# kernel-matrix-benchmarks/kernel-matrix-benchmarks

Measured on AMD Instinct MI355X. Metric: point-pair interactions/s (N*M/s) + max |err| vs scipy, D=3 Gaussian, higher is better.
Workload: dtype f32

## Files before the change

kernel_matrix_benchmarks_amd/csrc/kmvp_api.hip:

```cpp
#include "kmvp_ctx.hpp"

namespace kmvp {

Rccl g_rccl;

namespace {
thread_local std::string g_create_error;
}

int fail(kmvp_ctx* c, int code, const std::string& msg) {
  if (c) c->err = msg;
  else g_create_error = msg;
  return code;
}
const char* create_error() { return g_create_error.c_str(); }

int ensure(kmvp_ctx* c, DevBuf& b, size_t bytes) {
  if (bytes <= b.cap && b.p) return KMVP_OK;
  if (b.p) {
    HIP_TRY(c, hipFree(b.p));
    b.p = nullptr;
    b.cap = 0;
  }
  if (bytes == 0) bytes = 16;
// ... 237 lines not shown
  ncclResult_t r = g_rccl.GetUniqueId(&id);
  if (r != ncclSuccess) return fail(nullptr, KMVP_E_COMM, std::string("ncclGetUniqueId: ") + g_rccl.GetErrorString(r));
  memcpy(id128, &id, sizeof(id));
  return KMVP_OK;
}

int kmvp_comm_init(kmvp_ctx* c, const void* id128, int rank, int world) {
  if (!c || !id128 || world < 1 || rank < 0 || rank >= world) return fail(c, KMVP_E_INVALID, "bad communicator arguments");
  if (!g_rccl.load()) return fail(c, KMVP_E_COMM, g_rccl.error);
  HIP_TRY(c, hipSetDevice(c->device));
  if (c->comm) {
    g_rccl.CommDestroy(c->comm);
    c->comm = nullptr;
  }
  c->host_xchg = nullptr;
  c->host_user = nullptr;
  ncclUniqueId id;
  memcpy(&id, id128, sizeof(id));
  ncclResult_t r = g_rccl.CommInitRank(&c->comm, world, id, rank);
  if (r != ncclSuccess) {
    c->comm = nullptr;
    return fail(c, KMVP_E_COMM, std::string("ncclCommInitRank: ") + g_rccl.GetErrorString(r));
  }
  int count = -1, user_rank = -1, dev = -1;
  ncclResult_t r1 = g_rccl.CommCount(c->comm, &count);
  ncclResult_t r2 = g_rccl.CommUserRank(c->comm, &user_rank);
  (void)g_rccl.CommCuDevice(c->comm, &dev);
  if (r1 != ncclSuccess || r2 != ncclSuccess || count != world || user_rank != rank) {
    g_rccl.CommDestroy(c->comm);
    c->comm = nullptr;
    c->comm_count = 1;
    c->rank = 0;
    c->world = 1;
    return fail(c, KMVP_E_COMM, "RCCL communicator mismatch: asked for rank " + std::to_string(rank) + " of " +
                                    std::to_string(world) + " on device " + std::to_string(c->device) + ", RCCL reports rank " +
                                    std::to_string(user_rank) + " of " + std::to_string(count) + " on device " +
                                    std::to_string(dev));
  }
  c->comm_count = count;
  c->rank = rank;
  c->world = world;
  return KMVP_OK;
}

int kmvp_comm_init_host(kmvp_ctx* c, kmvp_host_allreduce_fn fn, void* user, int rank, int world) {
  if (!c || !fn || world < 1 || rank < 0 || rank >= world) return fail(c, KMVP_E_INVALID, "bad communicator arguments");
  if (c->comm) {
    g_rccl.CommDestroy(c->comm);
    c->comm = nullptr;
  }
  c->host_xchg = fn;
  c->host_user = user;
  c->comm_count = world;
  c->rank = rank;
  c->world = world;
  return KMVP_OK;
}

int kmvp_comm_world(const kmvp_ctx* c) { return (c && c->exchanges()) ? c->comm_count : 1; }
int kmvp_comm_rank(const kmvp_ctx* c) { return (c && c->exchanges()) ? c->rank : 0; }

int kmvp_set_option(kmvp_ctx* c, const char* key, int64_t value) {
  if (!c || !key) return KMVP_E_INVALID;
  const std::string k(key);
  if (k == "feed") {
    if (value < -1 || value > 1) return fail(c, KMVP_E_INVALID, "feed must be -1 (auto), 0 or 1");
    c->opt_feed = (int)value;
  } else if (k == "targets_per_lane") {
    if (value != 0 && value != 1 && value != 2 && value != 4 && value != 8)
      return fail(c, KMVP_E_INVALID, "targets_per_lane must be 0 (auto), 1, 2, 4 or 8");
    c->opt_T = (int)value;
  } else if (k == "segments") {
    if (value < 0 || value > 65535) return fail(c, KMVP_E_INVALID, "segments out of range");
    c->opt_segments = (int)value;
  } else if (k == "fast_sqdists") {
    if (value < -1 || value > 4) return fail(c, KMVP_E_INVALID, "fast_sqdists must be -1 (auto), 0, 1, 2, 3 or 4");
    c->opt_fast = (int)value;
  } else if (k == "cellmm_shape") {
    if (value < -1 || value > 1) return fail(c, KMVP_E_INVALID, "cellmm_shape must be -1 (by size), 0 (32x32x16) or 1 (16x16x32)");
    c->opt_cellmm_shape = (int)value;
  } else if (k == "cell_fused") {
    if (value < -1 || value > 1) return fail(c, KMVP_E_INVALID, "cell_fused must be -1 (automatic), 0 (two launches) or 1 (one launch where it applies)");
    c->opt_cell_fused = (int)value;
  } else if (k == "mfma_variant") {
    if (value != -1 && value != 0 && value != 1 && value != 4 && value != 5)
      return fail(c, KMVP_E_INVALID, "mfma_variant must be -1 (by kernel), 0, 1, 4 or 5");
    c->opt_mfma_variant = (int)value;
  } else if (k == "same_points_global") {
    c->opt_same_global = value != 0;
  } else if (k == "partial_shard") {
    c->opt_partial = value != 0;
  } else if (k == "fast_tiles") {
    if (value != 0 && value != 1 && value != 2 && value != 4 && value != 8)
      return fail(c, KMVP_E_INVALID, "fast_tiles must be 0 (auto), 1, 2, 4 or 8");
    c->opt_fast_tiles = (int)value;
  } else if (k == "chunk") {
    if (value < 8 || value > (1 << 24)) return fail(c, KMVP_E_INVALID, "chunk out of range");
    c->opt_chunk = (int)value;
  } else {
    return fail(c, KMVP_E_INVALID, "unknown option " + k);
  }
  return KMVP_OK;
}

int64_t kmvp_device_bytes(const kmvp_ctx* c) {
  if (!c) return 0;
  size_t t = 0;
  for (const DevBuf* b : {&c->y_raw, &c->x_raw, &c->b_raw, &c->xs, &c->rec, &c->x_scaled,
                          &c->y_scaled, &c->part, &c->partd, &c->aux, &c->sortbuf, &c->perm, &c->sums, &c->out, &c->scratch, &c->sdiag, &c->xchg, &c->kexp, &c->kshift, &c->xchgk, &c->kflag,
                    &c->sk_xs_x, &c->sk_rec_y, &c->sk_xs_y, &c->sk_rec_x, &c->sk_state,
                          &c->cell_tperm, &c->cell_sperm, &c->cell_tgrp, &c->cell_sgrp, &c->cell_slot, &c->cell_tmeta, &c->cell_sums, &c->cell_skey, &c->cell_scentre, &c->cell_scale})
    t += b->cap;
  return (int64_t)t;
}
double kmvp_last_kernel_ms(const kmvp_ctx* c) { return c ? c->last_kernel_ms : 0.0; }
double kmvp_last_total_ms(const kmvp_ctx* c) { return c ? c->last_total_ms : 0.0; }
double kmvp_last_allreduce_ms(const kmvp_ctx* c) { return c ? c->last_allreduce_ms : 0.0; }
const char* kmvp_last_kernel_name(const kmvp_ctx* c) { return c ? c->last_kernel_name : ""; }
const char* kmvp_last_dispatch_note(const kmvp_ctx* c) { return c ? c->note.c_str() : ""; }

}
```

kernel_matrix_benchmarks_amd/csrc/kmvp_cellmm.hpp:

```cpp
#pragma once
#include <hip/hip_runtime.h>
#include <stdint.h>

#include "kmvp_cell.hpp"

namespace kmvp {

#ifndef CMM_BF16
#define CMM_BF16 0
#endif
#if CMM_BF16
typedef __bf16 cmm_half;
#else
typedef _Float16 cmm_half;
#endif
typedef cmm_half f16x8 __attribute__((ext_vector_type(8)));
typedef cmm_half f16x2 __attribute__((ext_vector_type(2)));

constexpr int CMM_STAGE_TILES = 12;
constexpr int CMM_STAGE_BYTES = 8192;
constexpr int CMM_E_OFF = 0;
constexpr int CMM_B_OFF = CMM_STAGE_TILES * CELL_TILE * 16;
constexpr int CMM_HDR_OFF = CMM_B_OFF + CMM_STAGE_TILES * CELL_TILE * 4;
static_assert(CMM_HDR_OFF + CMM_STAGE_TILES * 16 <= CMM_STAGE_BYTES, "stage image too small");
constexpr float CMM_TARGET_SCALE = 64.f;
constexpr int CMM_MAX_WLOG2 = 8;

struct CellmmArgs {
  const float* xd;
  const float* tmeta;
  const unsigned char* img;
  const float* scale;
  double* part;
  int64_t n_slots;
  int64_t tile_base;
  int64_t m_stages;
  int64_t seg_stages;
  int segments;
  int tile_blocks;
};

typedef int i32x4 __attribute__((ext_vector_type(4)));

__device__ __forceinline__ f16x2 cellmm_pk(float a, float b) {
#if CMM_BF16
  f16x2 r;
  r[0] = (cmm_half)a;
  r[1] = (cmm_half)b;
  return r;
#else
  return __builtin_bit_cast(f16x2, __builtin_amdgcn_cvt_pkrtz(a, b));
#endif
}

__device__ __forceinline__ f16x8 cellmm_target_operand(const f32x4 d, int h) {
  float s[3], sh[3], sm[3];
#pragma unroll
  for (int c = 0; c < 3; ++c) {
    s[c] = d[c] * CMM_TARGET_SCALE;
    sh[c] = (float)(cmm_half)s[c];
    sm[c] = s[c] - sh[c];
  }
  const float q = CMM_TARGET_SCALE;
  float lo[8], hi[8];
  lo[0] = sh[0]; lo[1] = sh[1]; lo[2] = sh[0]; lo[3] = sh[1]; lo[4] = sm[0]; lo[5] = sm[1];
  lo[6] = d[0] * d[0] * (0.5f * q);
  lo[7] = d[1] * d[1] * (0.5f * q);
  hi[0] = sh[2]; hi[1] = d[0] * d[2] * q; hi[2] = sh[2]; hi[3] = d[0] * d[2] * q; hi[4] = sm[2];
  hi[5] = d[1] * d[2] * q;
  hi[6] = d[2] * d[2] * (0.5f * q);
  hi[7] = d[0] * d[1] * q;
  f16x8 out;
#pragma unroll
  for (int j = 0; j < 8; ++j) out[j] = (cmm_half)(h ? hi[j] : lo[j]);
  return out;
}

typedef float f32x2 __attribute__((ext_vector_type(2)));

template <int CTRL, int ROWMASK>
__device__ __forceinline__ float cellmm_dpp(float v) {
  return __int_as_float(__builtin_amdgcn_update_dpp(0, __float_as_int(v), CTRL, ROWMASK, 0xf, false));
}
__device__ __forceinline__ float cellmm_half_sum(float v) {
  v += cellmm_dpp<0x111, 0xf>(v);
  v += cellmm_dpp<0x112, 0xf>(v);
  v += cellmm_dpp<0x114, 0xf>(v);
  v += cellmm_dpp<0x118, 0xf>(v);
  v += cellmm_dpp<0x142, 0xa>(v);
  return __int_as_float(__builtin_amdgcn_readlane(__float_as_int(v), 31));
}
__device__ __forceinline__ float cellmm_cross_half_add(float v) {
  const auto r = __builtin_amdgcn_permlane32_swap(__float_as_int(v), __float_as_int(v), false, false);
  return __int_as_float(r[0]) + __int_as_float(r[1]);
}

template <int TT>
__global__ void __launch_bounds__(BLOCK_THREADS) __attribute__((amdgpu_waves_per_eu(TT >= 8 ? 2 : 1)))
cellmm_kernel(const CellmmArgs a) {
  constexpr int SB = CMM_STAGE_BYTES;
  constexpr int PIECES = SB / (16 * BLOCK_THREADS);
  constexpr float LOG2E = 1.4426950408889634f;
  __shared__ __attribute__((aligned(16))) unsigned char lds[2][SB];

  int tb, seg;
  block_to_work((int)blockIdx.x, a.segments, a.tile_blocks, tb, seg);
  const int lane = threadIdx.x & 63;
  const int wave = threadIdx.x >> 6;
  const int r = lane & 31;
  const int h = lane >> 5;
  const int64_t tile0 = a.tile_base + ((int64_t)tb * WAVES_PER_BLOCK + wave) * TT;

  constexpr bool HOLD_D = TT < 8;
  __shared__ __attribute__((aligned(16))) float dsh[HOLD_D ? 1 : WAVES_PER_BLOCK][HOLD_D ? 1 : TT][CELL_TILE][4];
  float dl[HOLD_D ? TT : 1][3], cT[3], U[TT];
  f16x8 xb[TT];
#pragma unroll
  for (int tt = 0; tt < TT; ++tt) {
    const f32x4 v = *reinterpret_cast<const f32x4*>(a.xd + ((tile0 + tt) * CELL_TILE + r) * 4);
    const f32x4 m = *reinterpret_cast<const f32x4*>(a.tmeta + (tile0 + tt) * 4);
#pragma unroll
    for (int c = 0; c < 3; ++c) {
// ... 81 lines not shown
      }
      U[tt] = kexp2(s2 * -LOG2E);
    }
  };

  for (int64_t s = s_begin; s < s_end; ++s) {
    const int buf = (int)((s - s_begin) & 1);
    if (s + 1 < s_end) fetch(s + 1);
    const unsigned char* base = &lds[buf][0];
    const unsigned char* p_ef = base + CMM_E_OFF + r * 16;
    const unsigned char* p_b = base + CMM_B_OFF + r * 4;
    const f32x4* hdr = reinterpret_cast<const f32x4*>(base + CMM_HDR_OFF);
#pragma unroll 1
    for (int q = 0; q < CMM_STAGE_TILES; ++q) {
      const f32x4 cs = hdr[q];
      const int ks = __builtin_amdgcn_readfirstlane(__float_as_int(cs[3]));
      if (ks < 0) break;
      if (ks != key_s) new_cell(cs, ks);
      const f32x4 ef = *reinterpret_cast<const f32x4*>(p_ef);
      const float bq = *reinterpret_cast<const float*>(p_b);
      p_ef += CELL_TILE * 16;
      p_b += CELL_TILE * 4;
      const f32x4 a14 = h ? f32x4{ef[2], ef[0] * ef[2], ef[2] * ef[2], ef[0] * ef[1]}
                          : f32x4{ef[0], ef[1], ef[0] * ef[0], ef[1] * ef[1]};
      const float a5 = h ? ef[1] * ef[2] : ef[1];
      const float arg = fmaf(ef[0], D1[0], fmaf(ef[1], D1[1], fmaf(ef[2], D1[2], ef[3])));
      const float wb = kexp2(arg) * bq;
      {
        const float yk = wb - S0c;
        const float tk = S0 + yk;
        S0c = (tk - S0) - yk;
        S0 = tk;
      }
      const float u1 = a14[0] * wb, u2 = a14[1] * wb;
      const f16x2 R0 = cellmm_pk(u1, u2);
      const float c1 = (float)R0[0], c2 = (float)R0[1];
      const f16x2 R1 = cellmm_pk(u1 - c1, u2 - c2);
      const f16x2 R3 = cellmm_pk(a14[2] * wb, a14[3] * wb);
      const f16x2 R2 = cellmm_pk(c1, a5 * wb);
      i32x4 yw;
      yw[0] = __builtin_bit_cast(int, R0);
      yw[1] = __builtin_bit_cast(int, R1);
      yw[2] = __builtin_bit_cast(int, R2);
      yw[3] = __builtin_bit_cast(int, R3);
      const f16x8 ya = __builtin_bit_cast(f16x8, yw);
#pragma unroll
      for (int tt = 0; tt < TT; ++tt) {
#if CMM_BF16
        acc[tt] = __builtin_amdgcn_mfma_f32_32x32x16_bf16(ya, xb[tt], acc[tt], 0, 0, 0);
#else
        acc[tt] = __builtin_amdgcn_mfma_f32_32x32x16_f16(ya, xb[tt], acc[tt], 0, 0, 0);
#endif
      }
    }
    if (s + 1 < s_end) commit(buf ^ 1);
    __syncthreads();
  }
  if (key_s >= 0) fold();

  const double inv = (double)a.scale[1];
#pragma unroll
  for (int tt = 0; tt < TT; ++tt)
    if (h == 0) a.part[(int64_t)seg * a.n_slots + (tile0 + tt - a.tile_base) * CELL_TILE + r] = outd[tt] * inv;
}


__device__ __forceinline__ float cellmm16_fold4(float a, float b, float c, float d) {
  const auto p = __builtin_amdgcn_permlane16_swap(__float_as_uint(a), __float_as_uint(b), false, false);
  const float w0 = __uint_as_float(p[0]) + __uint_as_float(p[1]);
  const auto q = __builtin_amdgcn_permlane16_swap(__float_as_uint(c), __float_as_uint(d), false, false);
  const float w1 = __uint_as_float(q[0]) + __uint_as_float(q[1]);
  const auto r = __builtin_amdgcn_permlane32_swap(__float_as_uint(w0), __float_as_uint(w1), false, false);
  return __uint_as_float(r[0]) + __uint_as_float(r[1]);
}
__device__ __forceinline__ float cellmm16_sources_sum(float v) {
  v += cellmm_dpp<0x111, 0xf>(v);
  v += cellmm_dpp<0x112, 0xf>(v);
  v += cellmm_dpp<0x114, 0xf>(v);
  v += cellmm_dpp<0x118, 0xf>(v);
  return __int_as_float(__builtin_amdgcn_readlane(__float_as_int(v), 15)) +
         __int_as_float(__builtin_amdgcn_readlane(__float_as_int(v), 47));
}

#ifndef CMM16_NOFOLD
#define CMM16_NOFOLD 0
#endif

template <int TT>
__device__ __forceinline__ void cellmm16_body(const CellmmArgs& a, int bid, unsigned char (*lds)[CMM_STAGE_BYTES]) {
  static_assert(!CMM_BF16, "f16 operands only");
  constexpr int SB = CMM_STAGE_BYTES;
  constexpr int PIECES = SB / (16 * BLOCK_THREADS);
  constexpr float LOG2E = 1.4426950408889634f;
  constexpr int HT = 2 * TT;
  constexpr int NG = (HT + 3) / 4;

  int tb, seg;
  block_to_work(bid, a.segments, a.tile_blocks, tb, seg);
  const int lane = threadIdx.x & 63;
  const int wave = threadIdx.x >> 6;
  const int cc = lane & 15;
  const int kg = lane >> 4;
  const int h = kg & 1;
  const int rs = 16 * (kg >> 1) + cc;
  const int64_t tile0 = a.tile_base + ((int64_t)tb * WAVES_PER_BLOCK + wave) * TT;

  float cT[3];
  f16x8 xb[HT];
#pragma unroll
  for (int u = 0; u < HT; ++u) {
    const f32x4 v = *reinterpret_cast<const f32x4*>(a.xd + ((tile0 + (u >> 1)) * CELL_TILE + 16 * (u & 1) + cc) * 4);
    xb[u] = cellmm_target_operand(v, h);
  }
  {
    const f32x4 m = *reinterpret_cast<const f32x4*>(a.tmeta + tile0 * 4);
#pragma unroll
    for (int c = 0; c < 3; ++c) cT[c] = __int_as_float(__builtin_amdgcn_readfirstlane(__float_as_int(m[c])));
  }
  float dl[NG][3], U[NG], vprev[NG];
  double outd[NG];
#pragma unroll
  for (int g = 0; g < NG; ++g) {
    const int u = 4 * g + kg < HT ? 4 * g + kg : HT - 1;
    const f32x4 v = *reinterpret_cast<const f32x4*>(a.xd + ((tile0 + (u >> 1)) * CELL_TILE + 16 * (u & 1) + cc) * 4);
#pragma unroll
    for (int c = 0; c < 3; ++c) dl[g][c] = v[c];
    U[g] = 0.f;
    vprev[g] = 0.f;
    outd[g] = 0.0;
  }

  f32x4 acc[HT];
#pragma unroll
  for (int u = 0; u < HT; ++u)
#pragma unroll
    for (int k = 0; k < 4; ++k) acc[u][k] = 0.f;

  const int64_t s_begin = (int64_t)seg * a.seg_stages;
  int64_t s_end = s_begin + a.seg_stages;
  if (s_end > a.m_stages) s_end = a.m_stages;

  f32x4 pre[PIECES];
  auto fetch = [&](int64_t s) {
    const unsigned char* src = a.img + s * SB;
#pragma unroll
    for (int p = 0; p < PIECES; ++p)
      pre[p] = *reinterpret_cast<const f32x4*>(src + (p * BLOCK_THREADS + (int)threadIdx.x) * 16);
  };
  auto commit = [&](int buf) {
#pragma unroll
    for (int p = 0; p < PIECES; ++p)
      *reinterpret_cast<f32x4*>(&lds[buf][(p * BLOCK_THREADS + (int)threadIdx.x) * 16]) = pre[p];
  };
  if (s_begin < s_end) {
    fetch(s_begin);
    commit(0);
  }
  __syncthreads();

  int key_s = -2;
  float S0 = 0.f, S0c = 0.f;
  float D1[3] = {0.f, 0.f, 0.f};

  auto fold = [&]() {
#if CMM16_NOFOLD
    asm volatile("" ::"v"(S0), "v"(S0c));
#else
    const float s0 = cellmm16_sources_sum(S0) * CMM_TARGET_SCALE;
    float x[4 * NG];
#pragma unroll
    for (int u = 0; u < 4 * NG; ++u) x[u] = u < HT ? (acc[u][0] + acc[u][1]) + (acc[u][2] + acc[u][3]) : 0.f;
#pragma unroll
    for (int g = 0; g < NG; ++g) {
      const float v = cellmm16_fold4(x[4 * g], x[4 * g + 1], x[4 * g + 2], x[4 * g + 3]);
      outd[g] += (double)(U[g] * ((v - vprev[g]) + s0));
      vprev[g] = v;
    }
#endif
    S0 = 0.f;
    S0c = 0.f;
  };
  auto new_cell = [&](const f32x4 cs, int ks) {
    if (key_s >= 0) fold();
    key_s = ks;
#pragma unroll
    for (int c = 0; c < 3; ++c) D1[c] = (cT[c] - cs[c]) * LOG2E;
#if !CMM16_NOFOLD
#pragma unroll
    for (int g = 0; g < NG; ++g) {
      float s2 = 0.f;
#pragma unroll
      for (int c = 0; c < 3; ++c) {
        const float df = dl[g][c] + (cT[c] - cs[c]);
        s2 = fmaf(df, df, s2);
      }
      U[g] = kexp2(s2 * -LOG2E);
    }
#endif
  };

  for (int64_t s = s_begin; s < s_end; ++s) {
    const int buf = (int)((s - s_begin) & 1);
    if (s + 1 < s_end) fetch(s + 1);
    const unsigned char* base = &lds[buf][0];
    const unsigned char* p_ef = base + CMM_E_OFF + rs * 16;
    const unsigned char* p_b = base + CMM_B_OFF + rs * 4;
    const f32x4* hdr = reinterpret_cast<const f32x4*>(base + CMM_HDR_OFF);
    const int keys = lane < CMM_STAGE_TILES ? __float_as_int(hdr[lane < CMM_STAGE_TILES ? lane : 0][3]) : -1;
#pragma unroll 1
    for (int q = 0; q < CMM_STAGE_TILES; ++q) {
      const int ks = __builtin_amdgcn_readlane(keys, q);
      if (ks < 0) break;
      if (ks != key_s) new_cell(hdr[q], ks);
      const f32x4 ef = *reinterpret_cast<const f32x4*>(p_ef);
      const float bq = *reinterpret_cast<const float*>(p_b);
      p_ef += CELL_TILE * 16;
      p_b += CELL_TILE * 4;
      const float m0 = h ? ef[2] : ef[0];
      const float m1 = h ? ef[0] : ef[1];
      const float m2 = h ? ef[2] : 1.f;
      const f32x4 a14 = f32x4{m0, m1 * m2, m0 * m0, m1 * ef[1]};
      const float a5 = ef[1] * m2;
      const float arg = fmaf(ef[0], D1[0], fmaf(ef[1], D1[1], fmaf(ef[2], D1[2], ef[3])));
      const float wb = kexp2(arg) * bq;
      {
        const float yk = wb - S0c;
        const float tk = S0 + yk;
        S0c = (tk - S0) - yk;
        S0 = tk;
      }
      const float u1 = a14[0] * wb, u2 = a14[1] * wb;
      const f16x2 R0 = cellmm_pk(u1, u2);
      const float c1 = (float)R0[0], c2 = (float)R0[1];
      const f16x2 R1 = cellmm_pk(u1 - c1, u2 - c2);
      const f16x2 R3 = cellmm_pk(a14[2] * wb, a14[3] * wb);
      const f16x2 R2 = cellmm_pk(c1, a5 * wb);
      i32x4 yw;
      yw[0] = __builtin_bit_cast(int, R0);
      yw[1] = __builtin_bit_cast(int, R1);
      yw[2] = __builtin_bit_cast(int, R2);
      yw[3] = __builtin_bit_cast(int, R3);
      const f16x8 ya = __builtin_bit_cast(f16x8, yw);
#pragma unroll
      for (int u = 0; u < HT; ++u) acc[u] = __builtin_amdgcn_mfma_f32_16x16x32_f16(ya, xb[u], acc[u], 0, 0, 0);
    }
    if (s + 1 < s_end) commit(buf ^ 1);
    __syncthreads();
  }
  if (key_s >= 0) fold();
#if CMM16_NOFOLD
#pragma unroll
  for (int u = 0; u < HT; ++u) asm volatile("" ::"v"(acc[u][0]), "v"(acc[u][1]), "v"(acc[u][2]), "v"(acc[u][3]));
#endif

  const double inv = (double)a.scale[1];
#pragma unroll
  for (int g = 0; g < NG; ++g)
    if (4 * g + kg < HT)
      a.part[(int64_t)seg * a.n_slots + (tile0 + 2 * g + (kg >> 1) - a.tile_base) * CELL_TILE + 16 * h + cc] = outd[g] * inv;
}

template <int TT>
__global__ void __launch_bounds__(BLOCK_THREADS) __attribute__((amdgpu_waves_per_eu(TT >= 8 ? 2 : 1)))
cellmm16_kernel(const CellmmArgs a, const CellmmArgs rest, const int main_grid) {
  __shared__ __attribute__((aligned(16))) unsigned char lds[2][CMM_STAGE_BYTES];
  if constexpr (TT > CELL_REST_TT) {
    const FusedCellWork w = fused_cell_work((int64_t)blockIdx.x, (int64_t)main_grid);
    if (w.list) {
      cellmm16_body<CELL_REST_TT>(rest, (int)w.local, lds);
      return;
    }
  }
  cellmm16_body<TT>(a, (int)blockIdx.x, lds);
}

hipError_t launch_cellmm_gaussian(int TT, int shape, const CellmmArgs& args, dim3 grid, hipStream_t stream, const char** kernel_name);
hipError_t launch_cellmm16_fused(int TT, const CellmmArgs& main, const CellmmArgs& rest, int64_t main_grid, int64_t rest_grid,
                                 hipStream_t stream, const char** kernel_name);

}
```

kernel_matrix_benchmarks_amd/csrc/kmvp_ctx.hpp:

```cpp
#pragma once
#include <dlfcn.h>
#include <hip/hip_runtime.h>
#include <rccl/rccl.h>
#include <stdint.h>
#include <stdlib.h>
#include <string.h>

#include <algorithm>
#include <cmath>
#include <string>
#include <vector>

#include "../../include/kmvp.h"
#include "kmvp_internal.hpp"

namespace kmvp {

enum : int { LAYOUT_LOWD = 0, LAYOUT_FAST = 1, LAYOUT_MFMA = 2, LAYOUT_CFAST = 3, LAYOUT_CELL = 4, LAYOUT_CELL64 = 5, LAYOUT_CELLMM = 6, LAYOUT_FASTMM = 7, LAYOUT_CFASTMM = 8 };

struct DevBuf {
  void* p = nullptr;
  size_t cap = 0;
};

// ... 20 lines not shown
      if (slash != std::string::npos) {
        const std::string dir = hip_path.substr(0, slash + 1);
        names.push_back(dir + "librccl.so.1");
        names.push_back(dir + "librccl.so");
      }
    }
    names.push_back("librccl.so.1");
    names.push_back("librccl.so");
    names.push_back("/opt/rocm/lib/librccl.so.1");
    for (const std::string& n : names) {
      handle = dlopen(n.c_str(), RTLD_NOW | RTLD_LOCAL);
      if (handle) {
        path = n;
        break;
      }
    }
    if (!handle) {
      error = std::string("cannot load librccl: ") + dlerror();
      return false;
    }
    GetUniqueId = (decltype(GetUniqueId))dlsym(handle, "ncclGetUniqueId");
    CommInitRank = (decltype(CommInitRank))dlsym(handle, "ncclCommInitRank");
    AllReduce = (decltype(AllReduce))dlsym(handle, "ncclAllReduce");
    CommDestroy = (decltype(CommDestroy))dlsym(handle, "ncclCommDestroy");
    GetErrorString = (decltype(GetErrorString))dlsym(handle, "ncclGetErrorString");
    CommCount = (decltype(CommCount))dlsym(handle, "ncclCommCount");
    CommUserRank = (decltype(CommUserRank))dlsym(handle, "ncclCommUserRank");
    CommCuDevice = (decltype(CommCuDevice))dlsym(handle, "ncclCommCuDevice");
    if (!GetUniqueId || !CommInitRank || !AllReduce || !CommDestroy || !GetErrorString || !CommCount || !CommUserRank ||
        !CommCuDevice) {
      error = "librccl lacks an expected symbol";
      return false;
    }
    return true;
  }
};extern Rccl g_rccl;

}

struct kmvp_ctx {
  using DevBuf = kmvp::DevBuf;
  int device = 0;
  hipStream_t stream = nullptr;
  hipEvent_t ev[5] = {nullptr, nullptr, nullptr, nullptr, nullptr};
  std::string err;

  int dtype = -1;
  int D = 0, E = 0;
  int64_t M = 0, N = 0, j_offset = 0, m_total = 0;
  bool same_points = false;
  bool have_points = false, have_signal = false, density = false;
  bool async_product = false;
  bool diag_on = false;
  int64_t diag_n = 0;
  double diag_ridge = 0.0, diag_min = 0.0;

  DevBuf y_raw, x_raw, b_raw;
  DevBuf xs, rec;
  DevBuf partd;
  DevBuf aux;
  DevBuf sortbuf, perm;
  DevBuf x_scaled, y_scaled;
  DevBuf cell_tperm, cell_sperm, cell_tgrp, cell_sgrp, cell_slot, cell_tmeta, cell_sums, cell_skey, cell_scentre, cell_scale;
  DevBuf part, sums, out;
  DevBuf xchg;
  DevBuf kexp, kshift, xchgk;
  DevBuf kflag;
  DevBuf scratch;
  DevBuf sdiag;
  DevBuf sk_xs_x, sk_rec_y, sk_xs_y, sk_rec_x, sk_state;
  uint64_t sk_points_ver = 0;
  uint64_t points_ver = 0, signal_ver = 0;
  int packed_layout = -1;
  int packed_kernel = -1, packed_sig = -1, packed_T = -1;
  uint64_t packed_points_ver = 0, packed_signal_ver = 0;
  int gen_kernel = -1;
  uint64_t gen_points_ver = 0;
  int64_t out_n = 0;
  int out_e = 0;

  int opt_feed = -1, opt_T = 0, opt_segments = 0, opt_chunk = 512;
  int opt_fast = -1, opt_fast_tiles = 0;
  int opt_cellmm_shape = -1;
  int opt_cell_fused = -1;
  int opt_mfma_variant = -1;
  int opt_same_global = 0;
  int opt_partial = 0;
  uint64_t perm_ver = 0;
  uint64_t cell_ver = 0;
  int cell_state = 0;
  int cell_tt = 0, cell_tt_req = 0;
  float cell_lo[3] = {0.f, 0.f, 0.f}, cell_hh[3] = {1.f, 1.f, 1.f};
  int cell_g[3] = {1, 1, 1};
  int64_t cell_n_tiles = 0, cell_m_tiles = 0;
  int64_t cell_n_main = 0, cell_n_rest = 0;
  float cloud_radius2 = INFINITY;
  uint64_t centre_ver = 0;

  ncclComm_t comm = nullptr;
  int rank = 0, world = 1;
  kmvp_host_allreduce_fn host_xchg = nullptr;
  void* host_user = nullptr;
  std::vector<double> host_buf;
  bool exchanges() const { return comm != nullptr || host_xchg != nullptr; }

  int comm_count = 1;
  float last_kernel_ms = 0.f, last_total_ms = 0.f, last_allreduce_ms = 0.f;
  const char* last_kernel_name = "";
  std::string note;
};

namespace kmvp {

int fail(kmvp_ctx* c, int code, const std::string& msg);
const char* create_error();

#define HIP_TRY(c, expr)                                                                     \
  do {                                                                                       \
    hipError_t e_ = (expr);                                                                  \
    if (e_ != hipSuccess)                                                                    \
      return kmvp::fail((c), e_ == hipErrorOutOfMemory ? KMVP_E_NOMEM : KMVP_E_DEVICE,       \
                        std::string(#expr) + ": " + hipGetErrorString(e_));                  \
  } while (0)

inline size_t elem_size(int dtype) { return dtype == KMVP_F64 ? 8 : 4; }
inline unsigned blocks_for(int64_t n, int threads = 256) { return (unsigned)((n + threads - 1) / threads); }

int ensure(kmvp_ctx* c, DevBuf& b, size_t bytes);
void release(DevBuf& b);

int run_product(kmvp_ctx* c, int kernel, bool normalise);
int measure_clouds(kmvp_ctx* c, int dtype, int64_t M, int64_t N, int D);
int prepare_points(kmvp_ctx* c, int kernel);
int run_gradient(kmvp_ctx* c, int kernel);
int run_logsumexp(kmvp_ctx* c, int kernel);
int run_logsumexp_grad(kmvp_ctx* c, int kernel);

int cg_solve(kmvp_ctx* c, int kernel, const void* a_host, int E, double rtol, int maxit, double* out_b,
             int* iters, double* resid);
int minres_solve(kmvp_ctx* c, int kernel, const void* a_host, int E, double rtol, int maxit,
                 double* out_b, int* iters, double* resid);

int sinkhorn_solve(kmvp_ctx* c, int kernel, const double* log_a, const double* log_b, double tol, int maxit, double* u,
                   double* v, int* iters, double* err);

}
```

kernel_matrix_benchmarks_amd/csrc/kmvp_plan.hpp:

```cpp
#pragma once
#include <algorithm>
#include <cstdint>
#include <vector>

namespace kmvp {

constexpr int WAVES_PER_BLOCK = 4;
constexpr int CELL_TILE = 32;
constexpr int CELL_REST_TT = 2;
constexpr int STAGED_TILE = 32;
constexpr int64_t SMALL_PROBLEM_TARGETS = 32768;
constexpr int SEG_SPLIT_FROM = 16;
constexpr int64_t MAX_GRID = 0x7fffffff;

inline int64_t round_up(int64_t v, int64_t q) { return (v + q - 1) / q * q; }
inline bool small_problem(int64_t N) { return N < SMALL_PROBLEM_TARGETS; }


struct SegmentRule {
  int64_t stage_bytes;
  int cols;
  int64_t min_seg = 1;
  bool small = false;
  int64_t l2_seg_bytes = 2 << 20;
// ... 115 lines not shown

inline void cell_split_count(const unsigned* keys, int64_t n, int TT, int64_t* n_main, int64_t* n_rest) {
  *n_main = *n_rest = 0;
  for_each_key_run(keys, n, [&](int64_t, int64_t cnt, unsigned) {
    const CellTiles s = split_cell_tiles((cnt + CELL_TILE - 1) / CELL_TILE, TT);
    *n_main += s.main_live + s.main_empty;
    *n_rest += s.rest_live + s.rest_empty;
  });
}

inline TileList cell_tiles_split(const unsigned* keys, int64_t n, int TT, int64_t* n_main, int64_t* n_rest) {
  TileList main, rest;
  main.reserve((size_t)n / 24 + 64);
  for_each_key_run(keys, n, [&](int64_t p, int64_t cnt, unsigned k) {
    const CellTiles s = split_cell_tiles((cnt + CELL_TILE - 1) / CELL_TILE, TT);
    main.add_cell(p, p, p + cnt, k, s.main_live, s.main_empty, CELL_TILE);
    rest.add_cell(p, p + s.main_live * CELL_TILE, p + cnt, k, s.rest_live, s.rest_empty, CELL_TILE);
  });
  main.pad_to((size_t)TT * WAVES_PER_BLOCK);
  rest.pad_to((size_t)CELL_REST_TT * WAVES_PER_BLOCK);
  *n_main = (int64_t)main.size();
  *n_rest = (int64_t)rest.size();
  main.append(rest);
  return main;
}

struct CellSplit {
  int64_t m_stages, n_slots;
  int64_t blocks[2], slots[2], seg_stages[2];
  int segments[2];
  int64_t grid(int r) const { return blocks[r] * segments[r]; }
  size_t region_offset(int cols, int r) const { return r ? (size_t)segments[0] * cols * slots[0] : 0; }
  size_t part_doubles(int cols) const { return ((size_t)segments[0] * slots[0] + (size_t)segments[1] * slots[1]) * cols; }
};

inline CellSplit cell_split(int64_t N, int64_t m_tiles, int64_t n_main, int64_t n_rest, int tt, int opt_segments,
                            int stage_tiles, SegmentRule main) {
  CellSplit s;
  main.small = small_problem(N);
  if (main.small) main.min_seg = 1;
  s.m_stages = (m_tiles + stage_tiles - 1) / stage_tiles;
  s.n_slots = (n_main + n_rest) * CELL_TILE;
  s.blocks[0] = n_main / (tt * WAVES_PER_BLOCK);
  s.blocks[1] = n_rest / (CELL_REST_TT * WAVES_PER_BLOCK);
  s.slots[0] = n_main * CELL_TILE;
  s.slots[1] = n_rest * CELL_TILE;
  s.segments[0] = stage_segments(opt_segments, std::max<int64_t>(1, s.blocks[0]), s.m_stages, s.n_slots, main);
  s.seg_stages[0] = (s.m_stages + s.segments[0] - 1) / s.segments[0];
  s.segments[1] = 0;
  s.seg_stages[1] = 1;
  if (s.blocks[1] > 0) {
    SegmentRule rest = main;
    rest.min_seg = 1;
    rest.target_blocks = 1536;
    const int seg = choose_segments(opt_segments, s.blocks[1], s.m_stages, s.n_slots, rest);
    s.seg_stages[1] = (s.m_stages + seg - 1) / seg;
    s.segments[1] = (int)((s.m_stages + s.seg_stages[1] - 1) / s.seg_stages[1]);
  }
  return s;
}


struct FusedCellWork {
  int list;
  int64_t local;
};
constexpr FusedCellWork fused_cell_work(int64_t bid, int64_t main_grid) {
  return bid < main_grid ? FusedCellWork{0, bid} : FusedCellWork{1, bid - main_grid};
}

struct FusedCellGrid {
  bool fused;
  int64_t main_grid, rest_grid, total;
};
inline FusedCellGrid fused_cell_grid(const CellSplit& s, int tt, int opt_fused) {
  FusedCellGrid g;
  g.main_grid = s.grid(0);
  g.rest_grid = s.grid(1);
  g.total = g.main_grid + g.rest_grid;
  g.fused = opt_fused != 0 && tt > CELL_REST_TT && s.blocks[1] > 0 && g.total <= MAX_GRID;
  return g;
}

}
```

kernel_matrix_benchmarks_amd/csrc/kmvp_product.hip:

```cpp
#include "kmvp_ctx.hpp"
#include <vector>
#include "kmvp_cell_pack.hpp"
#include "kmvp_cell64_pack.hpp"
#include "kmvp_cellmm_pack.hpp"
#include "kmvp_cfast_pack.hpp"
#include "kmvp_fast_pack.hpp"
#include "kmvp_fastmm_pack.hpp"
#include "kmvp_cfastmm_pack.hpp"
#include "kmvp_mfma_pack.hpp"

namespace kmvp {
namespace {

template <typename real>
hipError_t launch_lowd(int kernel, int D, int E, int sig, LowdTuning tune,
                       const LowdArgs<real>& args, dim3 grid, hipStream_t s, const char** name);
template <>
hipError_t launch_lowd<float>(int kernel, int D, int E, int sig, LowdTuning tune,
                              const LowdArgs<float>& args, dim3 grid, hipStream_t s,
                              const char** name) {
  switch (kernel) {
    case K_GAUSSIAN: return launch_lowd_gaussian_f32(D, E, sig, tune, args, grid, s, name);
    case K_ABSEXP: return launch_lowd_absexp_f32(D, E, sig, tune, args, grid, s, name);
    case K_INVDIST: return launch_lowd_invdist_f32(D, E, sig, tune, args, grid, s, name);
// ... 1337 lines not shown
  CellArgs a;
  a.xd = (const float*)c->xs.p;
  a.tmeta = (const float*)c->cell_tmeta.p;
  a.img = (const unsigned char*)c->rec.p;
  a.m_stages = m_stages;
  a.chunk_stages = std::max(1, c->opt_chunk / (CELL_TILE * CELL_STAGE_TILES));
  HIP_TRY(c, mark(c, 0));
  hipError_t le = hipSuccess;
  for (int r = 0; r < 2 && le == hipSuccess; ++r)
    if (s.blocks[r] > 0) {
      cell_args(c, s, NE, r, a);
      le = launch_cell_gaussian(sig, cell_tt(c, r), a, dim3((unsigned)s.grid(r)), c->stream, &c->last_kernel_name);
    }
  if (le == hipErrorInvalidValue) return fail(c, KMVP_E_UNSUPPORTED, "fast_tiles must be 1, 2, 4 or 8");
  HIP_TRY(c, le);
  HIP_TRY(c, mark(c, 1));

  if ((rc = ensure(c, c->sums, (size_t)NE * N * sizeof(double)))) return rc;
  if ((rc = ensure(c, c->cell_sums, (size_t)NE * n_slots * sizeof(double)))) return rc;
  for (int r = 0; r < 2; ++r)
    if (s.blocks[r] > 0)
      hipLaunchKernelGGL(reduce_region_kernel, dim3(blocks_for((int64_t)NE * s.slots[r])), dim3(256), 0, c->stream,
                         (const double*)cell_region(c, s, NE, r), (double*)c->cell_sums.p, s.slots[r], NE, s.segments[r], n_slots,
                         r ? s.slots[0] : (int64_t)0);
  hipLaunchKernelGGL(gather_cells_kernel, dim3(blocks_for((int64_t)NE * N)), dim3(256), 0, c->stream,
                     (const double*)c->cell_sums.p, (const int*)c->cell_slot.p, (double*)c->sums.p, N, n_slots, NE);
  HIP_TRY(c, hipGetLastError());
  return finish_product(c, (int64_t)NE * N, N, N, E, sig);
}


int cellmm_wlog2(const kmvp_ctx* c) {
  double arg = 0.0;
  for (int a = 0; a < c->D; ++a) arg += (double)c->cell_hh[a] * ((double)c->cell_g[a] * c->cell_hh[a]);
  return (int)std::ceil(arg * 1.4426950408889634);
}

int run_product_cellmm(kmvp_ctx* c, int sig) {
  const int D = c->D;
  const int E = sig == SIG_DENSITY ? 1 : c->E;
  const int NE = sig == SIG_NORM ? E + 1 : E;
  const int64_t N = c->N;
  const int TT = c->cell_tt;
  SegmentRule rule(CMM_STAGE_BYTES, 1);
  rule.min_seg = 2;
  rule.l2_seg_bytes = 3 << 20;
  rule.target_blocks = 7168;
  const CellSplit s = cell_plan(c, CMM_STAGE_TILES, rule);
  const int64_t m_stages = s.m_stages, n_slots = s.n_slots;
  int rc;
  CellGrid grid;
  cell_load_grid(c, grid);

  const PackKey key = {LAYOUT_CELLMM, K_GAUSSIAN, TT};
  const int image_sig = NE > 1 ? -1 : sig;
  const bool sig_stale = signal_stale(c, key, image_sig);
  const int* sgrp = (const int*)c->cell_sgrp.p;
  if ((rc = ensure(c, c->cell_scale, 64))) return rc;
  float* scale = (float*)c->cell_scale.p;
  unsigned* bmax = (unsigned*)c->cell_scale.p + 4;
  HIP_TRY(c, mark(c, 0));
  if (points_stale(c, key)) {
    if ((rc = pack_cell_targets(c, grid))) return rc;
    if ((rc = ensure(c, c->rec, (size_t)m_stages * CMM_STAGE_BYTES))) return rc;
    hipLaunchKernelGGL(pack_cellmm_points_kernel, dim3((unsigned)(m_stages * CMM_STAGE_TILES)), dim3(CELL_TILE), 0,
                       c->stream, (const float*)c->y_raw.p, (const int*)c->cell_sperm.p, sgrp, sgrp + c->cell_m_tiles,
                       (const unsigned*)(sgrp + 2 * c->cell_m_tiles), c->cell_m_tiles, D, grid, (unsigned char*)c->rec.p);
    HIP_TRY(c, hipGetLastError());
  }
  record_packed(c, key, image_sig);

  if ((rc = ensure(c, c->part, s.part_doubles(1) * sizeof(double)))) return rc;
  if ((rc = ensure(c, c->sums, (size_t)NE * N * sizeof(double)))) return rc;
  if ((rc = ensure(c, c->cell_sums, (size_t)NE * n_slots * sizeof(double)))) return rc;
  const int shape = c->opt_cellmm_shape >= 0 ? c->opt_cellmm_shape : ((TT >= 8 && c->N >= 500000 && c->M >= 100000) ? 1 : 0);
  FusedCellGrid fg = fused_cell_grid(s, TT, c->opt_cell_fused);
  if (shape != 1) fg.fused = false;
  CellmmArgs a;
  a.xd = (const float*)c->xs.p;
  a.tmeta = (const float*)c->cell_tmeta.p;
  a.img = (const unsigned char*)c->rec.p;
  a.scale = scale;
  a.m_stages = m_stages;
  if (NE == 1 && !sig_stale) HIP_TRY(c, mark(c, 0));
  for (int col = 0; col < NE; ++col) {
    if (sig_stale) {
      const float* b = (sig == SIG_DENSITY || col == E) ? (const float*)nullptr : (const float*)c->b_raw.p;
      HIP_TRY(c, hipMemsetAsync(bmax, 0, sizeof(unsigned), c->stream));
      if (b)
        hipLaunchKernelGGL(cellmm_absmax_kernel, dim3((unsigned)std::min<int64_t>(1024, (c->M + 255) / 256)), dim3(256), 0,
                           c->stream, b, c->M, E, col, bmax);
      hipLaunchKernelGGL(cellmm_scale_kernel, dim3(1), dim3(1), 0, c->stream, (const unsigned*)bmax, cellmm_wlog2(c),
                         b ? 0 : 1, scale);
      hipLaunchKernelGGL(pack_cellmm_signal_kernel, dim3((unsigned)(m_stages * CMM_STAGE_TILES)), dim3(CELL_TILE), 0,
                         c->stream, b, E, col, (const int*)c->cell_sperm.p, sgrp, sgrp + c->cell_m_tiles, c->cell_m_tiles,
                         (const float*)scale, (unsigned char*)c->rec.p);
      HIP_TRY(c, hipGetLastError());
      if (NE == 1) HIP_TRY(c, mark(c, 0));
    }
    hipError_t le = hipSuccess;
    if (fg.fused) {
      CellmmArgs ar = a;
      cell_args(c, s, 1, 0, a);
      cell_args(c, s, 1, 1, ar);
      le = launch_cellmm16_fused(TT, a, ar, fg.main_grid, fg.rest_grid, c->stream, &c->last_kernel_name);
    } else {
      for (int r = 0; r < 2 && le == hipSuccess; ++r)
        if (s.blocks[r] > 0) {
          cell_args(c, s, 1, r, a);
          le = launch_cellmm_gaussian(cell_tt(c, r), shape, a, dim3((unsigned)s.grid(r)), c->stream, &c->last_kernel_name);
        }
    }
    if (le == hipErrorInvalidValue) return fail(c, KMVP_E_UNSUPPORTED, "fast_tiles must be 1, 2, 4 or 8");
    HIP_TRY(c, le);
    if (NE == 1) HIP_TRY(c, mark(c, 1));
    double* col_sums = (double*)c->cell_sums.p + (size_t)col * n_slots;
    for (int r = 0; r < 2; ++r)
      if (s.blocks[r] > 0)
        hipLaunchKernelGGL(reduce_segments_kernel, dim3(blocks_for(s.slots[r])), dim3(256), 0, c->stream,
                           (const double*)cell_region(c, s, 1, r), col_sums + (r ? s.slots[0] : 0), s.slots[r], s.segments[r], 0);
    HIP_TRY(c, hipGetLastError());
  }
  if (NE > 1) HIP_TRY(c, mark(c, 1));

  hipLaunchKernelGGL(gather_cells_kernel, dim3(blocks_for((int64_t)NE * N)), dim3(256), 0, c->stream,
                     (const double*)c->cell_sums.p, (const int*)c->cell_slot.p, (double*)c->sums.p, N, n_slots, NE);
  HIP_TRY(c, hipGetLastError());
  return finish_product(c, (int64_t)NE * N, N, N, E, sig);
}


int cell64_prepare(kmvp_ctx* c) {
  if (c->cell_ver == c->points_ver && c->cell_state != 0) return KMVP_OK;
  c->cell_ver = c->points_ver;
  c->cell_state = -1;
  const int D = c->D;
  if (D > CELL_MAX_D || !(c->cloud_radius2 < INFINITY) || c->N > 0x3fffffff || c->M > 0x3fffffff) return KMVP_OK;
  float aux[FAST_AUX_FLOATS];
  HIP_TRY(c, hipMemcpyAsync(aux, c->aux.p, sizeof(aux), hipMemcpyDeviceToHost, c->stream));
  HIP_TRY(c, hipStreamSynchronize(c->stream));
  CellGrid grid;
  if (!cell_make_grid(aux, D, (float)((float)std::sqrt(2.0 * CELL64_T_MAX / (double)D)), grid)) return KMVP_OK;
  int rc;
  std::vector<unsigned> keys;
  if ((rc = cell_sort(c, c->y_raw.p, c->M, grid, c->cell_sperm, keys, &c->cell_skey))) return rc;
  std::vector<int> runs;
  std::vector<double> centres;
  for_each_key_run(keys.data(), c->M, [&](int64_t first, int64_t count, unsigned key) {
    runs.push_back((int)first);
    runs.push_back((int)count);
    for (int a = 0; a < 3; ++a) centres.push_back(a < D ? cell64_centre(key, a, grid) : 0.0);
    centres.push_back(0.0);
  });
  c->cell_m_tiles = (int64_t)runs.size() / 2;
  if ((rc = ensure(c, c->cell_sgrp, runs.size() * sizeof(int)))) return rc;
  if ((rc = ensure(c, c->cell_scentre, centres.size() * sizeof(double)))) return rc;
  HIP_TRY(c, hipMemcpyAsync(c->cell_sgrp.p, runs.data(), runs.size() * sizeof(int), hipMemcpyHostToDevice, c->stream));
  HIP_TRY(c, hipMemcpyAsync(c->cell_scentre.p, centres.data(), centres.size() * sizeof(double), hipMemcpyHostToDevice, c->stream));
  HIP_TRY(c, hipStreamSynchronize(c->stream));
  if (!c->same_points && (rc = cell_sort(c, c->x_raw.p, c->N, grid, c->cell_tperm, keys))) return rc;
  const TileList targets = cell_tiles(keys.data(), (int64_t)keys.size(), CELL64_TILE);
  if ((rc = upload_tiles(c, targets, c->cell_tgrp))) return rc;
  c->cell_n_tiles = (int64_t)targets.size();
  c->cell_tt = 1;
  cell_store_grid(c, grid);
  c->cell_state = 1;
// ... 569 lines not shown
```

Measured before the change: 42650 billion.

## Share MFMA source-operand build across waves in one-cell cellmm16 workgroups

When every wave in a workgroup targets the same cell, each wave now builds the f16 source operand (exp weight times signal and moments) for only its share of a stage's tiles. It writes the operand and weights to LDS, and all waves read them for their MFMAs, so the exp and packing work is no longer repeated per wave. Raw loads and the build are software-pipelined two stages ahead, and the header is kept in registers. This costs more LDS per block, adds a per-block one-cell check, and enables the shared path by default for tile counts of 8 and above.

After: 43670 billion (median of 6 runs). 1.02x the previous value.

```diff
diff --git a/kernel_matrix_benchmarks_amd/csrc/kmvp_api.hip b/kernel_matrix_benchmarks_amd/csrc/kmvp_api.hip
--- a/kernel_matrix_benchmarks_amd/csrc/kmvp_api.hip
+++ b/kernel_matrix_benchmarks_amd/csrc/kmvp_api.hip
@@ -343,6 +343,9 @@
   } else if (k == "cell_fused") {
     if (value < -1 || value > 1) return fail(c, KMVP_E_INVALID, "cell_fused must be -1 (automatic), 0 (two launches) or 1 (one launch where it applies)");
     c->opt_cell_fused = (int)value;
+  } else if (k == "cell_shared_build") {
+    if (value < -1 || value > 1) return fail(c, KMVP_E_INVALID, "cell_shared_build must be -1 (automatic), 0 (never) or 1 (wherever a workgroup is one-cell)");
+    c->opt_cell_shared_build = (int)value;
   } else if (k == "mfma_variant") {
     if (value != -1 && value != 0 && value != 1 && value != 4 && value != 5)
       return fail(c, KMVP_E_INVALID, "mfma_variant must be -1 (by kernel), 0, 1, 4 or 5");
diff --git a/kernel_matrix_benchmarks_amd/csrc/kmvp_cellmm.hpp b/kernel_matrix_benchmarks_amd/csrc/kmvp_cellmm.hpp
--- a/kernel_matrix_benchmarks_amd/csrc/kmvp_cellmm.hpp
+++ b/kernel_matrix_benchmarks_amd/csrc/kmvp_cellmm.hpp
@@ -38,6 +38,7 @@
   int64_t seg_stages;
   int segments;
   int tile_blocks;
+  int shared_build;
 };
 
 typedef int i32x4 __attribute__((ext_vector_type(4)));
@@ -285,18 +286,62 @@
          __int_as_float(__builtin_amdgcn_readlane(__float_as_int(v), 47));
 }
 
+__device__ __forceinline__ void cellmm16_operand(const f32x4 ef, float bq, float d1x, float d1y, float d1z, int h, f16x8& ya,
+                                                 float& wexp) {
+  const float m0 = h ? ef[2] : ef[0];
+  const float m1 = h ? ef[0] : ef[1];
+  const float m2 = h ? ef[2] : 1.f;
+  const f32x4 a14 = f32x4{m0, m1 * m2, m0 * m0, m1 * ef[1]};
+  const float a5 = ef[1] * m2;
+  const float arg = fmaf(ef[0], d1x, fmaf(ef[1], d1y, fmaf(ef[2], d1z, ef[3])));
+  wexp = kexp2(arg);
+  const float wb = wexp * bq;
+  const float u1 = a14[0] * wb, u2 = a14[1] * wb;
+  const f16x2 R0 = cellmm_pk(u1, u2);
+  const float c1 = (float)R0[0], c2 = (float)R0[1];
+  const f16x2 R1 = cellmm_pk(fmaf(a14[0], wb, -c1), fmaf(a14[1], wb, -c2));
+  const f16x2 R3 = cellmm_pk(a14[2] * wb, a14[3] * wb);
+  const f16x2 R2 = cellmm_pk(c1, a5 * wb);
+  i32x4 yw;
+  yw[0] = __builtin_bit_cast(int, R0);
+  yw[1] = __builtin_bit_cast(int, R1);
+  yw[2] = __builtin_bit_cast(int, R2);
+  yw[3] = __builtin_bit_cast(int, R3);
+  ya = __builtin_bit_cast(f16x8, yw);
+}
+__device__ __forceinline__ void cellmm16_weight_sum(float bq, float wexp, float& S0, float& S0c) {
+  const float yk = fmaf(bq, wexp, -S0c);
+  const float tk = S0 + yk;
+  S0c = (tk - S0) - yk;
+  S0 = tk;
+}
+
 #ifndef CMM16_NOFOLD
 #define CMM16_NOFOLD 0
 #endif
-
-template <int TT>
-__device__ __forceinline__ void cellmm16_body(const CellmmArgs& a, int bid, unsigned char (*lds)[CMM_STAGE_BYTES]) {
+#ifndef CMM16_BUILD_PROBE
+#define CMM16_BUILD_PROBE 0
+#endif
+
+constexpr int CMM16_ABUF_BYTES = CMM_STAGE_TILES * 64 * 16;
+constexpr int CMM16_WBUF_OFF = 2 * CMM16_ABUF_BYTES;
+constexpr int CMM16_WBUF_BYTES = CMM_STAGE_TILES * CELL_TILE * 8;
+constexpr int CMM16_SHARED_LDS_BYTES = CMM16_WBUF_OFF + 2 * CMM16_WBUF_BYTES;
+constexpr int CMM16_SHARED_OWN = CMM_STAGE_TILES / WAVES_PER_BLOCK;
+static_assert(CMM_STAGE_TILES % WAVES_PER_BLOCK == 0 && CMM_STAGE_TILES <= 64, "a stage's tiles: equal shares, one header lane each");
+constexpr bool cellmm16_has_shared(int TT) { return TT >= 8; }
+constexpr int cellmm16_lds_bytes(int TT) { return cellmm16_has_shared(TT) ? CMM16_SHARED_LDS_BYTES : 2 * CMM_STAGE_BYTES; }
+
+template <int TT, bool SHARED>
+__device__ __forceinline__ void cellmm16_body(const CellmmArgs& a, int bid, unsigned char* lds) {
   static_assert(!CMM_BF16, "f16 operands only");
+  static_assert(!SHARED || cellmm16_has_shared(TT), "no shared-build body at this tile count");
   constexpr int SB = CMM_STAGE_BYTES;
   constexpr int PIECES = SB / (16 * BLOCK_THREADS);
   constexpr float LOG2E = 1.4426950408889634f;
   constexpr int HT = 2 * TT;
   constexpr int NG = (HT + 3) / 4;
+  constexpr int OWN = CMM16_SHARED_OWN;
 
   int tb, seg;
   block_to_work(bid, a.segments, a.tile_blocks, tb, seg);
@@ -343,7 +388,7 @@
   int64_t s_end = s_begin + a.seg_stages;
   if (s_end > a.m_stages) s_end = a.m_stages;
 
-  f32x4 pre[PIECES];
+  f32x4 pre[SHARED ? 1 : PIECES];
   auto fetch = [&](int64_t s) {
     const unsigned char* src = a.img + s * SB;
 #pragma unroll
@@ -353,17 +398,64 @@
   auto commit = [&](int buf) {
 #pragma unroll
     for (int p = 0; p < PIECES; ++p)
-      *reinterpret_cast<f32x4*>(&lds[buf][(p * BLOCK_THREADS + (int)threadIdx.x) * 16]) = pre[p];
-  };
-  if (s_begin < s_end) {
-    fetch(s_begin);
-    commit(0);
+      *reinterpret_cast<f32x4*>(lds + buf * SB + (p * BLOCK_THREADS + (int)threadIdx.x) * 16) = pre[p];
+  };
+
+  const int wave_u = __builtin_amdgcn_readfirstlane(wave);
+  const int hl = lane < CMM_STAGE_TILES ? lane : 0;
+  f32x4 raw_ef[SHARED ? OWN : 1];
+  float raw_b[SHARED ? OWN : 1];
+  f32x4 hcur = {0.f, 0.f, 0.f, 0.f}, hnext = hcur, hfar = hcur;
+  auto load_hdr = [&](int64_t s) { return *reinterpret_cast<const f32x4*>(a.img + s * SB + CMM_HDR_OFF + hl * 16); };
+  auto load_raw = [&](int64_t s, int j) {
+    const unsigned char* src = a.img + s * SB;
+    const int row = (wave_u * OWN + j) * CELL_TILE + rs;
+    raw_ef[j] = *reinterpret_cast<const f32x4*>(src + CMM_E_OFF + row * 16);
+    raw_b[j] = *reinterpret_cast<const float*>(src + CMM_B_OFF + row * 4);
+  };
+  auto build_tile = [&](int buf, const f32x4 hd, int j) {
+    const int t = wave_u * OWN + j;
+    if (__builtin_amdgcn_readlane(__float_as_int(hd[3]), t) < 0) return;
+    float d1[3];
+#pragma unroll
+    for (int c = 0; c < 3; ++c)
+      d1[c] = (cT[c] - __int_as_float(__builtin_amdgcn_readlane(__float_as_int(hd[c]), t))) * LOG2E;
+    f16x8 ya;
+    float wexp;
+    cellmm16_operand(raw_ef[j], raw_b[j], d1[0], d1[1], d1[2], h, ya, wexp);
+    *reinterpret_cast<f16x8*>(lds + buf * CMM16_ABUF_BYTES + (t * 64 + lane) * 16) = ya;
+    if (h == 0)
+      *reinterpret_cast<f32x2*>(lds + CMM16_WBUF_OFF + buf * CMM16_WBUF_BYTES + (t * CELL_TILE + rs) * 8) = f32x2{raw_b[j], wexp};
+  };
+
+  if constexpr (SHARED) {
+    if (s_begin < s_end) {
+      hcur = load_hdr(s_begin);
+#pragma unroll
+      for (int j = 0; j < OWN; ++j) load_raw(s_begin, j);
+#pragma unroll
+      for (int j = 0; j < OWN; ++j) build_tile(0, hcur, j);
+      if (s_begin + 1 < s_end) {
+        hnext = load_hdr(s_begin + 1);
+#pragma unroll
+        for (int j = 0; j < OWN; ++j) load_raw(s_begin + 1, j);
+      }
+    }
+  } else {
+    if (s_begin < s_end) {
+      fetch(s_begin);
+      commit(0);
+    }
   }
   __syncthreads();
 
   int key_s = -2;
   float S0 = 0.f, S0c = 0.f;
   float D1[3] = {0.f, 0.f, 0.f};
+#if CMM16_BUILD_PROBE
+  f16x8 ya_probe = {};
+  float wexp_probe = 0.f;
+#endif
 
   auto fold = [&]() {
 #if CMM16_NOFOLD
@@ -404,50 +496,76 @@
 
   for (int64_t s = s_begin; s < s_end; ++s) {
     const int buf = (int)((s - s_begin) & 1);
-    if (s + 1 < s_end) fetch(s + 1);
-    const unsigned char* base = &lds[buf][0];
-    const unsigned char* p_ef = base + CMM_E_OFF + rs * 16;
-    const unsigned char* p_b = base + CMM_B_OFF + rs * 4;
-    const f32x4* hdr = reinterpret_cast<const f32x4*>(base + CMM_HDR_OFF);
-    const int keys = lane < CMM_STAGE_TILES ? __float_as_int(hdr[lane < CMM_STAGE_TILES ? lane : 0][3]) : -1;
+    if constexpr (SHARED) {
+      if (s + 1 < s_end) {
+#pragma unroll
+        for (int j = 0; j < OWN; ++j) build_tile(buf ^ 1, hnext, j);
+      }
+      if (s + 2 < s_end) {
+        hfar = load_hdr(s + 2);
+#pragma unroll
+        for (int j = 0; j < OWN; ++j) load_raw(s + 2, j);
+      }
+      const unsigned char* p_ya = lds + buf * CMM16_ABUF_BYTES + lane * 16;
+      const unsigned char* p_w = lds + CMM16_WBUF_OFF + buf * CMM16_WBUF_BYTES + rs * 8;
+      const int keys = lane < CMM_STAGE_TILES ? __float_as_int(hcur[3]) : -1;
 #pragma unroll 1
-    for (int q = 0; q < CMM_STAGE_TILES; ++q) {
-      const int ks = __builtin_amdgcn_readlane(keys, q);
-      if (ks < 0) break;
-      if (ks != key_s) new_cell(hdr[q], ks);
-      const f32x4 ef = *reinterpret_cast<const f32x4*>(p_ef);
-      const float bq = *reinterpret_cast<const float*>(p_b);
-      p_ef += CELL_TILE * 16;
-      p_b += CELL_TILE * 4;
-      const float m0 = h ? ef[2] : ef[0];
-      const float m1 = h ? ef[0] : ef[1];
-      const float m2 = h ? ef[2] : 1.f;
-      const f32x4 a14 = f32x4{m0, m1 * m2, m0 * m0, m1 * ef[1]};
-      const float a5 = ef[1] * m2;
-      const float arg = fmaf(ef[0], D1[0], fmaf(ef[1], D1[1], fmaf(ef[2], D1[2], ef[3])));
-      const float wb = kexp2(arg) * bq;
-      {
-        const float yk = wb - S0c;
-        const float tk = S0 + yk;
-        S0c = (tk - S0) - yk;
-        S0 = tk;
-      }
-      const float u1 = a14[0] * wb, u2 = a14[1] * wb;
-      const f16x2 R0 = cellmm_pk(u1, u2);
-      const float c1 = (float)R0[0], c2 = (float)R0[1];
-      const f16x2 R1 = cellmm_pk(u1 - c1, u2 - c2);
-      const f16x2 R3 = cellmm_pk(a14[2] * wb, a14[3] * wb);
-      const f16x2 R2 = cellmm_pk(c1, a5 * wb);
-      i32x4 yw;
-      yw[0] = __builtin_bit_cast(int, R0);
-      yw[1] = __builtin_bit_cast(int, R1);
-      yw[2] = __builtin_bit_cast(int, R2);
-      yw[3] = __builtin_bit_cast(int, R3);
-      const f16x8 ya = __builtin_bit_cast(f16x8, yw);
-#pragma unroll
-      for (int u = 0; u < HT; ++u) acc[u] = __builtin_amdgcn_mfma_f32_16x16x32_f16(ya, xb[u], acc[u], 0, 0, 0);
-    }
-    if (s + 1 < s_end) commit(buf ^ 1);
+      for (int q = 0; q < CMM_STAGE_TILES; ++q) {
+        const int ks = __builtin_amdgcn_readlane(keys, q);
+        if (ks < 0) break;
+        if (ks != key_s) {
+          f32x4 cs;
+#pragma unroll
+          for (int c = 0; c < 3; ++c) cs[c] = __int_as_float(__builtin_amdgcn_readlane(__float_as_int(hcur[c]), q));
+          cs[3] = 0.f;
+          new_cell(cs, ks);
+        }
+        const f16x8 ya = *reinterpret_cast<const f16x8*>(p_ya);
+        const f32x2 w = *reinterpret_cast<const f32x2*>(p_w);
+        p_ya += 64 * 16;
+        p_w += CELL_TILE * 8;
+        cellmm16_weight_sum(w[0], w[1], S0, S0c);
+#pragma unroll
+        for (int u = 0; u < HT; ++u) acc[u] = __builtin_amdgcn_mfma_f32_16x16x32_f16(ya, xb[u], acc[u], 0, 0, 0);
+      }
+      hcur = hnext;
+      hnext = hfar;
+    } else {
+      if (s + 1 < s_end) fetch(s + 1);
+      const unsigned char* base = lds + buf * SB;
+      const unsigned char* p_ef = base + CMM_E_OFF + rs * 16;
+      const unsigned char* p_b = base + CMM_B_OFF + rs * 4;
+      const f32x4* hdr = reinterpret_cast<const f32x4*>(base + CMM_HDR_OFF);
+      const int keys = lane < CMM_STAGE_TILES ? __float_as_int(hdr[hl][3]) : -1;
+#pragma unroll 1
+      for (int q = 0; q < CMM_STAGE_TILES; ++q) {
+        const int ks = __builtin_amdgcn_readlane(keys, q);
+        if (ks < 0) break;
+        if (ks != key_s) new_cell(hdr[q], ks);
+        const f32x4 ef = *reinterpret_cast<const f32x4*>(p_ef);
+        const float bq = *reinterpret_cast<const float*>(p_b);
+        p_ef += CELL_TILE * 16;
+        p_b += CELL_TILE * 4;
+#if CMM16_BUILD_PROBE
+        if ((q & 3) == wave_u) {
+          cellmm16_operand(ef, bq, D1[0], D1[1], D1[2], h, ya_probe, wexp_probe);
+        } else {
+          asm volatile("" ::"v"(ef[0]), "v"(ef[1]), "v"(ef[2]), "v"(ef[3]));
+        }
+        asm volatile("" ::"v"(bq), "v"(S0));
+        const f16x8 ya = ya_probe;
+        const float wexp = wexp_probe;
+#else
+        f16x8 ya;
+        float wexp;
+        cellmm16_operand(ef, bq, D1[0], D1[1], D1[2], h, ya, wexp);
+#endif
+        cellmm16_weight_sum(bq, wexp, S0, S0c);
+#pragma unroll
+        for (int u = 0; u < HT; ++u) acc[u] = __builtin_amdgcn_mfma_f32_16x16x32_f16(ya, xb[u], acc[u], 0, 0, 0);
+      }
+      if (s + 1 < s_end) commit(buf ^ 1);
+    }
     __syncthreads();
   }
   if (key_s >= 0) fold();
@@ -464,17 +582,36 @@
 }
 
 template <int TT>
+__device__ __forceinline__ bool cellmm16_one_cell(const CellmmArgs& a, int bid) {
+  int tb, seg;
+  block_to_work(bid, a.segments, a.tile_blocks, tb, seg);
+  const int* m = reinterpret_cast<const int*>(a.tmeta) + (a.tile_base + (int64_t)tb * WAVES_PER_BLOCK * TT) * 4;
+  int differ = 0;
+#pragma unroll
+  for (int w = 1; w < WAVES_PER_BLOCK; ++w)
+#pragma unroll
+    for (int c = 0; c < 3; ++c) differ |= m[(int64_t)w * TT * 4 + c] ^ m[c];
+  return __builtin_amdgcn_readfirstlane(differ) == 0;
+}
+
+template <int TT>
 __global__ void __launch_bounds__(BLOCK_THREADS) __attribute__((amdgpu_waves_per_eu(TT >= 8 ? 2 : 1)))
 cellmm16_kernel(const CellmmArgs a, const CellmmArgs rest, const int main_grid) {
-  __shared__ __attribute__((aligned(16))) unsigned char lds[2][CMM_STAGE_BYTES];
+  __shared__ __attribute__((aligned(16))) unsigned char lds[cellmm16_lds_bytes(TT)];
   if constexpr (TT > CELL_REST_TT) {
     const FusedCellWork w = fused_cell_work((int64_t)blockIdx.x, (int64_t)main_grid);
     if (w.list) {
-      cellmm16_body<CELL_REST_TT>(rest, (int)w.local, lds);
+      cellmm16_body<CELL_REST_TT, false>(rest, (int)w.local, lds);
       return;
     }
   }
-  cellmm16_body<TT>(a, (int)blockIdx.x, lds);
+  if constexpr (cellmm16_has_shared(TT)) {
+    if (a.shared_build && cellmm16_one_cell<TT>(a, (int)blockIdx.x)) {
+      cellmm16_body<TT, true>(a, (int)blockIdx.x, lds);
+      return;
+    }
+  }
+  cellmm16_body<TT, false>(a, (int)blockIdx.x, lds);
 }
 
 hipError_t launch_cellmm_gaussian(int TT, int shape, const CellmmArgs& args, dim3 grid, hipStream_t stream, const char** kernel_name);
diff --git a/kernel_matrix_benchmarks_amd/csrc/kmvp_ctx.hpp b/kernel_matrix_benchmarks_amd/csrc/kmvp_ctx.hpp
--- a/kernel_matrix_benchmarks_amd/csrc/kmvp_ctx.hpp
+++ b/kernel_matrix_benchmarks_amd/csrc/kmvp_ctx.hpp
@@ -126,6 +126,7 @@
   int opt_feed = -1, opt_T = 0, opt_segments = 0, opt_chunk = 512;
   int opt_fast = -1, opt_fast_tiles = 0;
   int opt_cellmm_shape = -1;
+  int opt_cell_shared_build = -1;
   int opt_cell_fused = -1;
   int opt_mfma_variant = -1;
   int opt_same_global = 0;
diff --git a/kernel_matrix_benchmarks_amd/csrc/kmvp_plan.hpp b/kernel_matrix_benchmarks_amd/csrc/kmvp_plan.hpp
--- a/kernel_matrix_benchmarks_amd/csrc/kmvp_plan.hpp
+++ b/kernel_matrix_benchmarks_amd/csrc/kmvp_plan.hpp
@@ -221,4 +221,20 @@
   return g;
 }
 
-}
+
+constexpr int CELL_SHARED_TT = 8;
+
+constexpr bool cell_shared_build(int tt, int opt) { return opt != 0 && tt >= CELL_SHARED_TT; }
+
+inline int64_t count_one_cell_blocks(const unsigned* keys, int64_t n_main, int tt) {
+  const int64_t per_block = (int64_t)tt * WAVES_PER_BLOCK;
+  int64_t one = 0;
+  for (int64_t t = 0; t + per_block <= n_main; t += per_block) {
+    bool same = true;
+    for (int w = 1; w < WAVES_PER_BLOCK; ++w) same = same && keys[t + (int64_t)w * tt] == keys[t];
+    one += same ? 1 : 0;
+  }
+  return one;
+}
+
+}
diff --git a/kernel_matrix_benchmarks_amd/csrc/kmvp_product.hip b/kernel_matrix_benchmarks_amd/csrc/kmvp_product.hip
--- a/kernel_matrix_benchmarks_amd/csrc/kmvp_product.hip
+++ b/kernel_matrix_benchmarks_amd/csrc/kmvp_product.hip
@@ -1443,6 +1443,7 @@
   a.img = (const unsigned char*)c->rec.p;
   a.scale = scale;
   a.m_stages = m_stages;
+  a.shared_build = cell_shared_build(TT, c->opt_cell_shared_build) ? 1 : 0;
   if (NE == 1 && !sig_stale) HIP_TRY(c, mark(c, 0));
   for (int col = 0; col < NE; ++col) {
     if (sig_stale) {
```
